# CapAI/ship-sim-gym

Hardware: AMD Instinct MI355X
Metric: env steps/sec (batched ShipEnv) (higher is better)
Workload: dtype f64

## Files before the change

ship_sim_gym_amd/csrc/shipsim_kernels.hip:

```cpp
#include <hip/hip_runtime.h>

#include <cfloat>
#include <cstdint>
#include <type_traits>

#include "shipsim.h"
#include "shipsim_internal.h"

namespace ssg {

__device__ __forceinline__ double *lds_base()
{
    extern __shared__ double s_lds[];
    return s_lds;
}

__device__ __forceinline__ double dmin(double a, double b) { return __builtin_fmin(a, b); }
__device__ __forceinline__ double dmax(double a, double b) { return __builtin_fmax(a, b); }

__device__ __forceinline__ double obs_fma(double a, double b, double c)
{
#ifndef SSG_NO_LIDAR_FMA
    return __builtin_fma(a, b, c);
#else
// ... 104 lines not shown
        const double py = goal_at<LDS_BANK, DYN>(c, goff, g, 1);
        const double dx = px - x, dy = py - y;
        const double d = obs_fma(dx, dx, dy * dy);
        const bool take = ((gm >> g) & 1u) & (d < best);
        best = take ? d : best;
        gi = take ? g : gi;
    }
    if (gi >= 0) { gx = goal_at<LDS_BANK, DYN>(c, goff, gi, 0); gy = goal_at<LDS_BANK, DYN>(c, goff, gi, 1); }
}

__device__ __forceinline__ void nearest_goal_regs(int n_goals, unsigned gm, double x, double y, const double *gp, double &gx, double &gy)
{
    gx = -1.0;
    gy = -1.0;
    double best = INFINITY;
#pragma unroll
    for (int g = 0; g < SSG_MAX_GOALS; ++g) {
        const double px = gp[2 * g], py = gp[2 * g + 1];
        const double dx = px - x, dy = py - y;
        const double d = obs_fma(dx, dx, dy * dy);
        const bool take = (g < n_goals) & (bool)((gm >> g) & 1u) & (d < best);
        best = take ? d : best;
        gx = take ? px : gx;
        gy = take ? py : gy;
    }
}

__device__ __forceinline__ int next_map(const DevCfg &c, int map_id, int env)
{
    if (c.map_ring > 0) {
        const int base = env * c.map_ring;
        const int nxt = map_id + 1;
        return (nxt - base >= c.map_ring) ? base : nxt;
    }
    const int nxt = map_id + 1;
    return (nxt >= c.n_maps) ? 0 : nxt;
}

__device__ __forceinline__ void beam_end(double cx, double cy, double ca, double sa, double cphi, double sphi, double dist,
                                         double &ex, double &ey)
{
    const double ux = obs_fma(ca, cphi, -(sa * sphi)), uy = obs_fma(sa, cphi, ca * sphi);
    ex = obs_fma(dist, ux, cx);
    ey = obs_fma(dist, uy, cy);
}

__host__ __device__ __forceinline__ constexpr int nb_lo(int nb) { return (nb + 1) / 2; }
constexpr int kBeamTabBytes = 2 * SSG_MAX_BEAMS * 8;
constexpr int kShipTabBytes = 6 * 8 * 8;
constexpr int kTrafficTabBytes = SSG_N_TRAFFIC * 4 * 8 * 8;
constexpr int kPoseDoubles = 7;
constexpr int kGoalScratchBytes = 64 * SSG_MAX_GOALS * 2 + 64 * 4;
constexpr int kTrafficScratchBytes = 64 * SSG_N_TRAFFIC * 2 + 64 * 4;
__host__ __device__ __forceinline__ constexpr int lds_fixed_bytes(int epw, bool dyn)
{
    return kBeamTabBytes + kShipTabBytes + (dyn ? kTrafficTabBytes : 0) + kPoseDoubles * epw * 8 + (dyn ? 8 : 6) * epw * 4 + 4 * (epw / 64) * 4 +
           (epw / 64) * (kGoalScratchBytes + (dyn ? kTrafficScratchBytes : 0));
}
__host__ __device__ __forceinline__ constexpr int lds_res_bytes(int nb) { return nb * 64 * 8; }
__host__ __device__ __forceinline__ constexpr int lds_queue_bytes(int nb0) { return (2 * nb0 * 64 + 64) * 2; }
__host__ __device__ __forceinline__ constexpr int lds_tile_bytes(int nb)
{
    return 2 * lds_res_bytes(nb) + 2 * lds_queue_bytes(nb_lo(nb));
}

constexpr int kHdrLidar = 10, kHdrGoals = 2 * SSG_MAX_GOALS;
static_assert(SSG_MAP_OFF_COUNTS == 0 && SSG_MAP_OFF_AABB == 2 && SSG_MAP_OFF_GOALS == kHdrLidar && SSG_MAP_OFF_SPAWN_GOAL == kHdrLidar + kHdrGoals,
              "the record's head: counts, boxes, goals, spawn goal");
#ifndef SSG_SIX_ROLE_MAX_EPW
#define SSG_SIX_ROLE_MAX_EPW 128
#endif
__host__ __device__ __forceinline__ constexpr int tile_roles(int epw, bool dyn) { return (epw <= SSG_SIX_ROLE_MAX_EPW && !dyn) ? 6 : 4; }
__host__ __device__ __forceinline__ constexpr int lds_hdr_bytes(int epw, bool lds_bank, bool dyn) { return lds_bank ? 0 : ((tile_roles(epw, dyn) - 2) * kHdrLidar + kHdrGoals) * epw * 8; }

constexpr unsigned long long kLidarMiss = ~0ull;

template <bool LDS_BANK> struct PlaneChunk { static constexpr int n = LDS_BANK ? 4 : 8; };

template <bool EXACT>
__device__ __forceinline__ double seg_mad(double a, double b, double c) { return EXACT ? a * b + c : obs_fma(a, b, c); }

template <bool LDS_BANK, bool EXACT>
__device__ __forceinline__ void lidar_pass(const DevCfg &c, const int n_items, const unsigned short *queue,
                                           unsigned long long *res , const double *beamtab,
                                           const double cx, const double cy, const double ca, const double sa,
                                           const int rec_off, const int lane, const double *hLt = nullptr , const int ld = 0)
{
    for (int base = 0; base < n_items; base += 64) {
        const int idx = base + lane;
        const bool act = idx < n_items;
        const unsigned code = queue[act ? idx : 0];
        const int src = code & 63, bi = (code >> 6) & (SSG_MAX_BEAMS - 1), s = (code >> 10) & 1;
        const double wcx = __shfl(cx, src), wcy = __shfl(cy, src), wca = __shfl(ca, src), wsa = __shfl(sa, src);
        const int woff = __shfl(rec_off, src);
        double ex, ey;
        beam_end(wcx, wcy, wca, wsa, beamtab[bi], beamtab[SSG_MAX_BEAMS + bi], c.lidar_dist, ex, ey);
        int cnt;
        if constexpr (LDS_BANK) cnt = (int)bank_at<LDS_BANK>(c, woff + SSG_MAP_OFF_COUNTS + s);
        else cnt = (int)hLt[s * ld + src];
        const int pb = woff + SSG_MAP_OFF_PLANES + s * (SSG_MAX_HULL * SSG_PLANE_DOUBLES);
        bool outside = false;
        bool out_sure = false, maybe = false;
        constexpr double kSignEps = 1e-9;
        bool ok = false;
        double ptx = ex, pty = ey;
        double bd = -1.0, bden = 1.0, t_hit = 0.0;
        int bj = 0;
        constexpr int kPlaneChunk = PlaneChunk<LDS_BANK>::n;
        for (int j0 = 0; __any(act & (j0 < cnt)); j0 += kPlaneChunk) {
            double pv0x[kPlaneChunk], pv0y[kPlaneChunk], pnx[kPlaneChunk], pny[kPlaneChunk], pv0n[kPlaneChunk];
            double pdtmin[kPlaneChunk], pdtmax[kPlaneChunk];
#pragma unroll
            for (int u = 0; u < kPlaneChunk; ++u) {
                const int j = j0 + u;
                const int q = pb + SSG_PLANE_DOUBLES * ((j < SSG_MAX_HULL) ? j : 0);
                const bool want = LDS_BANK || (act & (j < cnt));
                pv0x[u] = pv0y[u] = pnx[u] = pny[u] = pv0n[u] = 0.0;
                if (EXACT && want) { const double2 vv = bank_at2<LDS_BANK>(c, q + 0); pv0x[u] = vv.x; pv0y[u] = vv.y; }
                if (want) { const double2 nn = bank_at2<LDS_BANK>(c, q + 2); pnx[u] = nn.x; pny[u] = nn.y; }
                if (want) pv0n[u] = bank_at<LDS_BANK>(c, q + 4);
                if (EXACT) {
                    const int jp = (j == 0) ? cnt - 1 : j - 1;
                    const int qp = pb + SSG_PLANE_DOUBLES * ((jp >= 0 && jp < SSG_MAX_HULL) ? jp : 0);
                    const double ux = bank_at<LDS_BANK>(c, qp + 0), uy = bank_at<LDS_BANK>(c, qp + 1);
                    pdtmin[u] = seg_mad<EXACT>(pnx[u], uy, -(pny[u] * ux));
// ... 463 lines not shown
            const bool frontB = (snx_ * v0x + sny_ * v0y) > off_i;
            const unsigned long long mV = __ballot(valid);
            const unsigned long long mA = __ballot(valid & frontA);
            const unsigned long long missB = mV & ~__ballot(valid & frontB);
            const unsigned long long P = 0x0084210842108421ull;
            const unsigned long long allA = mA & (mA >> 1) & (mA >> 2) & (mA >> 3) & (mA >> 4) & P;
            bool sepB = false;
#pragma unroll
            for (int i = 0; i < SSG_SHIP_VERTS; ++i) sepB = sepB | (((missB >> i) & P) == 0ull);
            const bool separated = (allA != 0ull) | sepB;
            col = col | !separated;
        }
        colliding = (lane == src) ? col : colliding;
    }
    return colliding;
}

template <int NB, int EPW, bool LDS_BANK, bool EXACT, bool DYN>
__global__ __launch_bounds__(tile_roles(EPW, DYN) * EPW) void step_kernel(const DevCfg c, const int32_t *__restrict__ actions_kn,
                                                       double *__restrict__ obs, double *__restrict__ reward_out,
                                                       uint8_t *__restrict__ done_out, uint8_t *__restrict__ flags_out,
                                                       const int K_launch, const long long traj)
{
    const int K = DYN ? 1 : K_launch;
    SSG_CLOCK_BEGIN();
    constexpr int NB0 = nb_lo(NB);
    constexpr int NR = tile_roles(EPW, DYN);
    const int role = threadIdx.x / EPW;
    const int tl = threadIdx.x - role * EPW;
    const int e = blockIdx.x * EPW + tl;
    const bool live = e < c.n_envs;
    const int el_ = live ? e : 0;
    const size_t np = (size_t)c.n_pad;
    const int lane = threadIdx.x & 63;

    double *__restrict__ colX = c.f64cols + COL_X * np;
    double *__restrict__ colY = c.f64cols + COL_Y * np;
    double *__restrict__ colVX = c.f64cols + COL_VX * np;
    double *__restrict__ colVY = c.f64cols + COL_VY * np;
    double *__restrict__ colA = c.f64cols + COL_A * np;
    double *__restrict__ colW = c.f64cols + COL_W * np;
    double *__restrict__ colCum = c.f64cols + COL_CUM * np;
    double *__restrict__ colLid = c.f64cols + COL_LIDAR * np;
    int32_t *__restrict__ colRud = c.i32cols + ICOL_RUDDER * np;
    int32_t *__restrict__ colStep = c.i32cols + ICOL_STEP * np;
    int32_t *__restrict__ colMap = c.i32cols + ICOL_MAP * np;

    const int bank_bytes = LDS_BANK ? ((c.n_maps * (SSG_MAP_STRIDE * 8) + 15) & ~15) : 0;
    char *lds_fixed = reinterpret_cast<char *>(lds_base()) + bank_bytes;
    double *beamtab = reinterpret_cast<double *>(lds_fixed);
    double *shiptab = reinterpret_cast<double *>(lds_fixed + kBeamTabBytes);
    double *traffictab = reinterpret_cast<double *>(lds_fixed + kBeamTabBytes + kShipTabBytes);
    double *pose = reinterpret_cast<double *>(lds_fixed + kBeamTabBytes + kShipTabBytes + (DYN ? kTrafficTabBytes : 0));
    int *posem = reinterpret_cast<int *>(pose + kPoseDoubles * EPW);
    int *poser = posem + EPW;
    unsigned *gres = reinterpret_cast<unsigned *>(poser + EPW);
    unsigned *gdone = gres + 2 * EPW;
    unsigned *gtraf = gdone + 2 * EPW;
    unsigned *sync_ready = gtraf + (DYN ? 2 * EPW : 0);
    unsigned *sync_ack = sync_ready + EPW / 64;
    unsigned *sync_bar = sync_ack + EPW / 64;
    char *goal_scratch0 = reinterpret_cast<char *>(sync_bar + 2 * (EPW / 64));
    char *traffic_scratch0 = goal_scratch0 + (EPW / 64) * kGoalScratchBytes;
    char *scratch0 = lds_fixed + lds_fixed_bytes(EPW, DYN);
    char *tile_base = scratch0 + (tl >> 6) * lds_tile_bytes(NB);
    double *hdr0 = reinterpret_cast<double *>(scratch0 + (EPW / 64) * lds_tile_bytes(NB));
    double *hL = LDS_BANK ? nullptr : hdr0 + ((role & 1) + (role >= 4 ? 2 : 0)) * (kHdrLidar * EPW) + tl;
    double *hG = LDS_BANK ? nullptr : hdr0 + (NR - 2) * kHdrLidar * EPW + tl;
    auto load_hdr_lidar = [&](int rec_off) {
#pragma unroll
        for (int f = 0; f < kHdrLidar / 2; ++f) { const double2 v = bank_at2<LDS_BANK>(c, rec_off + 2 * f); hL[(2 * f) * EPW] = v.x; hL[(2 * f + 1) * EPW] = v.y; }
    };
    auto load_hdr_goals = [&](int rec_off) {
#pragma unroll
        for (int f = 0; f < kHdrGoals / 2; ++f) { const double2 v = bank_at2<LDS_BANK>(c, rec_off + SSG_MAP_OFF_GOALS + 2 * f); hG[(2 * f) * EPW] = v.x; hG[(2 * f + 1) * EPW] = v.y; }
    };

#ifdef SSG_STAMPS
    unsigned long long stamp_[16] = {};
#endif
    SSG_STAMP(8);

    double bank_tail_v = 0.0;
    int bank_tail_o = -1;
    if (LDS_BANK && !SSG_ABL(8)) stage_bank_lds<NR * EPW>(c.bank, c.n_maps * (SSG_MAP_STRIDE * 8), bank_tail_v, bank_tail_o);
    double tv[6] = {0.0, 0.0, 0.0, 0.0, 0.0, 0.0};
    if (threadIdx.x < 2 * SSG_MAX_BEAMS)
        tv[0] = (threadIdx.x < SSG_MAX_BEAMS) ? c.beam_cos[threadIdx.x & (SSG_MAX_BEAMS - 1)] : c.beam_sin[threadIdx.x & (SSG_MAX_BEAMS - 1)];
    if (threadIdx.x >= 64 && threadIdx.x < 64 + SSG_SHIP_VERTS) {
        const int i = threadIdx.x - 64, ip = (i == 0) ? (SSG_SHIP_VERTS - 1) : (i - 1);
        tv[0] = c.hull[2 * i]; tv[1] = c.hull[2 * i + 1]; tv[2] = c.nrm[2 * i]; tv[3] = c.nrm[2 * i + 1]; tv[4] = c.hull[2 * ip]; tv[5] = c.hull[2 * ip + 1];
    }
    if constexpr (DYN) {
        if (threadIdx.x >= 160 && threadIdx.x < 160 + SSG_N_TRAFFIC * SSG_SHIP_VERTS) {
            const int kk = (threadIdx.x - 160) / SSG_SHIP_VERTS, i = (threadIdx.x - 160) % SSG_SHIP_VERTS;
            tv[0] = c.thull[kk][2 * i]; tv[1] = c.thull[kk][2 * i + 1]; tv[2] = c.tnrm[kk][2 * i]; tv[3] = c.tnrm[kk][2 * i + 1];
        }
    }
    auto flush_tables = [&]() {
        if (bank_tail_o >= 0) *reinterpret_cast<double *>(reinterpret_cast<char *>(lds_base()) + bank_tail_o) = bank_tail_v;
        if (threadIdx.x < 2 * SSG_MAX_BEAMS) beamtab[threadIdx.x] = tv[0];
        if (threadIdx.x >= 64 && threadIdx.x < 64 + SSG_SHIP_VERTS) {
            const int i = threadIdx.x - 64;
            shiptab[0 * 8 + i] = tv[0]; shiptab[1 * 8 + i] = tv[1];
            shiptab[2 * 8 + i] = tv[2]; shiptab[3 * 8 + i] = tv[3];
            shiptab[4 * 8 + i] = tv[4]; shiptab[5 * 8 + i] = tv[5];
        }
        if constexpr (DYN) {
            if (threadIdx.x >= 160 && threadIdx.x < 160 + SSG_N_TRAFFIC * SSG_SHIP_VERTS) {
                const int kk = (threadIdx.x - 160) / SSG_SHIP_VERTS, i = (threadIdx.x - 160) % SSG_SHIP_VERTS;
                traffictab[(kk * 4 + 0) * 8 + i] = tv[0]; traffictab[(kk * 4 + 1) * 8 + i] = tv[1];
                traffictab[(kk * 4 + 2) * 8 + i] = tv[2]; traffictab[(kk * 4 + 3) * 8 + i] = tv[3];
            }
        }
    };
    if (threadIdx.x == 128) {
        double bl = INFINITY, br = -INFINITY, bb = INFINITY, bt = -INFINITY;
        for (int i = 0; i < SSG_SHIP_VERTS; ++i) {
            const double hx = c.hull[2 * i], hy = c.hull[2 * i + 1];
            const double wx = 1.0 * hx + (-0.0) * hy + c.spawn_x, wy = 0.0 * hx + 1.0 * hy + c.spawn_y;
            bl = dmin(bl, wx); br = dmax(br, wx); bb = dmin(bb, wy); bt = dmax(bt, wy);
        }
        shiptab[0 * 8 + 6] = c.spawn_x + (br - bl) / 2;
        shiptab[1 * 8 + 6] = c.spawn_y + (bt - bb) / 2;
    }
    if (threadIdx.x >= 192 && threadIdx.x < 192 + 4 * (EPW / 64)) sync_ready[threadIdx.x - 192] = 0u;
    const bool auto_reset = (c.flags & SSG_FLAG_AUTO_RESET) != 0u;
    const int tile = tl >> 6;
    auto wait_pose = [&](int k) {
        while (__hip_atomic_load(&sync_ready[tile], __ATOMIC_ACQUIRE, __HIP_MEMORY_SCOPE_WORKGROUP) != (unsigned)(k + 1))
            __builtin_amdgcn_s_sleep(2);
    };
    auto ack_pose = [&]() {
        if (lane == 0) __hip_atomic_fetch_add(&sync_ack[tile], 1u, __ATOMIC_RELEASE, __HIP_MEMORY_SCOPE_WORKGROUP);
    };
    unsigned *sync_q = sync_bar + EPW / 64;
    auto query_done = [&]() {
        if (lane == 0) __hip_atomic_fetch_add(&sync_q[tile], 1u, __ATOMIC_RELEASE, __HIP_MEMORY_SCOPE_WORKGROUP);
    };
    auto wait_queries = [&]() {
        while (__hip_atomic_load(&sync_q[tile], __ATOMIC_ACQUIRE, __HIP_MEMORY_SCOPE_WORKGROUP) < 2u)
            __builtin_amdgcn_s_sleep(1);
    };
    auto tile_barrier = [&](int k) {
        if (lane == 0) __hip_atomic_fetch_add(&sync_bar[tile], 1u, __ATOMIC_RELEASE, __HIP_MEMORY_SCOPE_WORKGROUP);
        while (__hip_atomic_load(&sync_bar[tile], __ATOMIC_ACQUIRE, __HIP_MEMORY_SCOPE_WORKGROUP) < (unsigned)NR * (unsigned)(k + 1))
            __builtin_amdgcn_s_sleep(1);
    };

    auto traffic_collide = [&](auto k0_, auto k1_, const double *tpre, double x, double y, double ca, double sa, int part,
                               unsigned short *tq , unsigned *tw ) {
        constexpr int K0 = decltype(k0_)::value, K1 = decltype(k1_)::value;
        const int wq = lane / 5, wi = lane - 5 * wq;
        const double w_hx = shiptab[0 * 8 + wi], w_hy = shiptab[1 * 8 + wi], w_nx = shiptab[2 * 8 + wi], w_ny = shiptab[3 * 8 + wi];
        double sbl, sbr, sbb, sbt;
        {
            double swx[SSG_SHIP_VERTS], swy[SSG_SHIP_VERTS];
            ship_world(shiptab, ca, sa, x, y, swx, swy, sbl, sbr, sbb, sbt);
        }
        tw[lane] = 0u;
        int n_tp = 0;
#pragma unroll
        for (int kk = K0; kk < K1; ++kk) {
            const double tx = tpre[4 * kk + 0], ty = tpre[4 * kk + 1];
            const double dx = dmax(dmax(sbl - tx, tx - sbr), 0.0), dy = dmax(dmax(sbb - ty, ty - sbt), 0.0);
            bool cand = false;
            if (live & ((dx * dx + dy * dy) <= c.dyn_reach2[kk])) {
                const double tca = tpre[4 * kk + 2], tsa = tpre[4 * kk + 3];
                double bl = INFINITY, br = -INFINITY, bb = INFINITY, bt = -INFINITY;
#pragma unroll
                for (int i = 0; i < SSG_SHIP_VERTS; ++i) {
                    const double gx = traffictab[(kk * 4 + 0) * 8 + i], gy = traffictab[(kk * 4 + 1) * 8 + i];
                    const double wx = tca * gx + (-tsa) * gy + tx, wy = tsa * gx + tca * gy + ty;
                    bl = dmin(bl, wx); br = dmax(br, wx); bb = dmin(bb, wy); bt = dmax(bt, wy);
                }
                cand = (sbl <= br) & (bl <= sbr) & (sbb <= bt) & (bb <= sbt);
            }
            const unsigned long long m = __ballot(cand);
            const int pos = n_tp + (int)__builtin_amdgcn_mbcnt_hi((unsigned)(m >> 32), __builtin_amdgcn_mbcnt_lo((unsigned)m, 0u));
            if (cand) tq[pos] = (unsigned short)(lane | (kk << 6));
            n_tp += __popcll(m);
        }
        for (int base = 0; base < n_tp; base += 12) {
            const int p = base + wq;
            const bool valid = (lane < 60) & (p < n_tp);
            const unsigned code = tq[valid ? p : 0];
            const int src = code & 63, kk = code >> 6;
            const double bx = __shfl(x, src), by = __shfl(y, src), bca = __shfl(ca, src), bsa = __shfl(sa, src);
            double tx = __shfl(tpre[4 * K0 + 0], src), ty = __shfl(tpre[4 * K0 + 1], src), tca = __shfl(tpre[4 * K0 + 2], src), tsa = __shfl(tpre[4 * K0 + 3], src);
#pragma unroll
            for (int h = K0 + 1; h < K1; ++h) {
                const double a0 = __shfl(tpre[4 * h + 0], src), a1 = __shfl(tpre[4 * h + 1], src);
                const double a2 = __shfl(tpre[4 * h + 2], src), a3 = __shfl(tpre[4 * h + 3], src);
                tx = (kk == h) ? a0 : tx; ty = (kk == h) ? a1 : ty; tca = (kk == h) ? a2 : tca; tsa = (kk == h) ? a3 : tsa;
            }
            const double *tt = traffictab + kk * 32;
            bool sep;
            {
                const double nx = bca * w_nx + (-bsa) * w_ny, ny = bsa * w_nx + bca * w_ny;
                const double vx_ = bca * w_hx + (-bsa) * w_hy + bx, vy_ = bsa * w_hx + bca * w_hy + by;
                const double off = nx * vx_ + ny * vy_;
                double mn = INFINITY;
// ... 25 lines not shown
        }
        gtraf[part * EPW + tl] = (tw[lane] != 0u) ? 1u : 0u;
    };
    auto traffic_hit = [&](int) -> unsigned { return gtraf[tl] | gtraf[EPW + tl]; };
    if (role < 2) {
        unsigned short *queue = reinterpret_cast<unsigned short *>(tile_base + 2 * lds_res_bytes(NB) + role * lds_queue_bytes(NB0));
        const int b_first = role ? NB0 : 0, b_count = role ? (NB - NB0) : NB0;
        double ca, sa, cx, cy;
        int map_id;
        double tpre[DYN ? 4 * SSG_N_TRAFFIC : 1] = {};
        {
            const double x = colX[el_], y = colY[el_], ang = colA[el_];
            map_id = colMap[el_];
            if constexpr (!LDS_BANK) load_hdr_lidar(map_id * SSG_MAP_STRIDE);
            { const double2 sc = sincos_call(ang); sa = sc.x; ca = sc.y; }
            if (role == 0) { pose[2 * EPW + tl] = ca; pose[3 * EPW + tl] = sa; }
            flush_tables();
            if (LDS_BANK) __builtin_amdgcn_s_waitcnt(0);
            __syncthreads();
            SSG_STAMP(9);
            if constexpr (DYN) {
                {
                    const double *tcol = c.dyn_f64 + (size_t)DC_TRAFFIC * np, *trot = c.dyn_f64 + (size_t)DC_TROT * np;
#pragma unroll
                    for (int kk = 0; kk < SSG_N_TRAFFIC; ++kk) {
                        if ((kk == 0) != (role == 0)) continue;
                        tpre[4 * kk + 0] = tcol[(size_t)(9 * kk) * np + el_]; tpre[4 * kk + 1] = tcol[(size_t)(9 * kk + 1) * np + el_];
                        tpre[4 * kk + 2] = trot[(size_t)(2 * kk) * np + el_]; tpre[4 * kk + 3] = trot[(size_t)(2 * kk + 1) * np + el_];
                    }
                }
            }
            double swx[SSG_SHIP_VERTS], swy[SSG_SHIP_VERTS], bl, br, bb, bt;
            ship_world(shiptab, ca, sa, x, y, swx, swy, bl, br, bb, bt);
            cx = x + (br - bl) / 2;
            cy = y + (bt - bb) / 2;
        }
        lidar_query<NB, LDS_BANK, EXACT>(c, reinterpret_cast<unsigned long long *>(tile_base), queue, beamtab, b_first, b_count,
                                         cx, cy, ca, sa, map_id * SSG_MAP_STRIDE, live, lane, hL, EPW);
        if (K == 1) query_done();
        for (int k = 0; k < K; ++k) {
            if constexpr (NR == 4) wait_pose(k);
            if constexpr (DYN) {
#pragma unroll
                for (int i = 0; i < 4 * SSG_N_TRAFFIC; ++i) asm volatile("" : "+v"(tpre[i]));
            }
            SSG_STAMP_K(0);
            double nca = 0.0, nsa = 0.0, ncx = 0.0, ncy = 0.0, npx = 0.0, npy = 0.0;
            int nmap = 0;
            if constexpr (NR == 4) {
                nca = pose[2 * EPW + tl]; nsa = pose[3 * EPW + tl];
                ncx = pose[4 * EPW + tl]; ncy = pose[5 * EPW + tl];
                npx = pose[0 * EPW + tl]; npy = pose[1 * EPW + tl];
                nmap = posem[tl];
                ack_pose();
                reinterpret_cast<unsigned short *>(gres)[2 * ((k & 1) * EPW + tl) + role] =
                        bank_narrowphase<LDS_BANK>(c, shiptab, npx, npy, nca, nsa, nmap * SSG_MAP_STRIDE, live, lane, role, hL, EPW) ? 1 : 0;
            }
            SSG_STAMP_K(4);
            if constexpr (DYN) {
                static_assert(lds_queue_bytes(1) >= 64 * 2 + 64 * 4, "lidar-lo's pair queue holds ship 0's pair queue and hit words");
                unsigned short *tq1 = reinterpret_cast<unsigned short *>(traffic_scratch0 + (tl >> 6) * kTrafficScratchBytes);
                if (role == 0) traffic_collide(std::integral_constant<int, 0>{}, std::integral_constant<int, 1>{}, tpre, npx, npy, nca, nsa, 0,
                                               queue, reinterpret_cast<unsigned *>(queue + 64));
                else traffic_collide(std::integral_constant<int, 1>{}, std::integral_constant<int, SSG_N_TRAFFIC>{}, tpre, npx, npy, nca, nsa, 1,
                                     tq1, reinterpret_cast<unsigned *>(tq1 + 64 * SSG_N_TRAFFIC));
            }

            SSG_STAMP_K(3);
            tile_barrier(k);
            SSG_STAMP_K(1);
            if constexpr (NR == 6) {
                if (k + 1 < K) {
                    nca = pose[2 * EPW + tl]; nsa = pose[3 * EPW + tl];
                    ncx = pose[4 * EPW + tl]; ncy = pose[5 * EPW + tl];
                    nmap = posem[tl];
                    ack_pose();
                }
            }
            if (k + 1 < K) {
                const bool rs = auto_reset & ((gres[(k & 1) * EPW + tl] | (gdone[(k & 1) * EPW + tl] & 1u) | (DYN ? traffic_hit(k) : 0u)) != 0u);
                ca = rs ? 1.0 : nca; sa = rs ? 0.0 : nsa;
                cx = rs ? shiptab[0 * 8 + 6] : ncx; cy = rs ? shiptab[1 * 8 + 6] : ncy;
                map_id = rs ? next_map(c, nmap, el_) : nmap;
                if constexpr (!LDS_BANK) {
                    if (rs) load_hdr_lidar(map_id * SSG_MAP_STRIDE);
                }
                lidar_query<NB, LDS_BANK, EXACT>(c, reinterpret_cast<unsigned long long *>(tile_base + ((k + 1) & 1) * lds_res_bytes(NB)),
                                                 queue, beamtab, b_first, b_count, cx, cy, ca, sa, map_id * SSG_MAP_STRIDE, live, lane, hL, EPW);
                if (k + 1 == K - 1) query_done();
            }
            SSG_STAMP_K(2);
        }
        if (K == 1 && live) {
            const bool rs = auto_reset & ((gres[tl] | (gdone[tl] & 1u) | (DYN ? traffic_hit(0) : 0u)) != 0u);
            const unsigned long long *rk = reinterpret_cast<const unsigned long long *>(tile_base);
            for (int kb = 0; kb < b_count; ++kb) {
                const int i = b_first + kb;
                const unsigned long long key = rk[i * 64 + lane];
                const double hitd = __longlong_as_double((long long)(key & 0x7FFFFFFFFFFFFFFFull));
                if (rs | (key != kLidarMiss)) st_out(&colLid[(size_t)i * np + el_], rs ? -1.0 : hitd);
            }
        }
        SSG_STAMP(10);
        SSG_STAMP_FLUSH(3);
        SSG_CLOCK_END();
        return;
    }

    if constexpr (NR == 6) {
// ... 56 lines not shown
            for (int i = 0; i < NB; ++i) asm volatile("" : "+v"(pv[6 + i]));
            if constexpr (DYN) asm volatile("" : "+v"(pv[4]), "+v"(pv[5]));
            int map0_ = map0; unsigned gm0_ = gm0;
            asm volatile("" : "+v"(map0_), "+v"(gm0_));
            gm_pre = gm0_;
            flush_tables();
            if (LDS_BANK) __builtin_amdgcn_s_waitcnt(0);
            __syncthreads();
            SSG_STAMP(9);
            if constexpr (!DYN)
                nearest_goal<LDS_BANK, false>(c, map0_ * SSG_MAP_STRIDE + SSG_MAP_OFF_GOALS, gm0_, pv[0], pv[1], pv[4], pv[5], hG, EPW);
        }
        const bool hist2 = c.history >= 2;
        ObsTile<NB> ot;
        ot.init(lane);
        constexpr int kObsPasses = (2 * F + ObsTile<NB>::CP - 1) / ObsTile<NB>::CP;
        constexpr bool kPairs = (NB >= 8) && (NB % 2 == 0);
        constexpr bool kSplitOk = kPairs || (F % ObsTile<NB>::CP) == 0;
        const bool split_last = kSplitOk && hist2 && c.history == 2 && !SSG_ABL(7);
        for (int k = 0; k < K; ++k) {
            const bool early = split_last && (k == K - 1);
            if constexpr (kSplitOk) {
                if (early) {
                    int tw = __builtin_amdgcn_readfirstlane(tl >> 6);
                    int te0 = blockIdx.x * EPW + 64 * tw;
                    asm volatile("" : "+s"(tw), "+s"(te0));
                    double *colbuf = reinterpret_cast<double *>(scratch0 + tw * lds_tile_bytes(NB) + ((k + 1) & 1) * lds_res_bytes(NB));
                    double *__restrict__ ob = obs + ((size_t)te0 + (size_t)k * (size_t)traj) * (size_t)(2 * F);
                    if constexpr (kPairs)
                        write_obs_pairs<NB, true, 0, F>(colbuf, [&](int j) -> double { return pv[(j < F) ? j : 0]; }, ob, min(64, c.n_envs - te0), lane);
                    else
                        write_obs_tile<NB, true, 0, F / ObsTile<NB>::CP>(ot, colbuf, [&](int j) -> double { return pv[(j < F) ? j : 0]; }, ob,
                                                                        min(64, c.n_envs - te0), lane);
                }
            }
            if constexpr (DYN) {
#pragma unroll
                for (int g = 0; g < SSG_MAX_GOALS; ++g) {
                    const bool listed = g < c.n_goals;
                    ogp[2 * g] = listed ? goal_at<LDS_BANK, DYN>(c, el_, g, 0) : 0.0;
                    ogp[2 * g + 1] = listed ? goal_at<LDS_BANK, DYN>(c, el_, g, 1) : 0.0;
                }
            }
            wait_pose(k);
            if constexpr (DYN) {
#pragma unroll
                for (int g = 0; g < 2 * SSG_MAX_GOALS; ++g) asm volatile("" : "+v"(ogp[g]));
            }
            SSG_STAMP_K(0);
            const double x = pose[0 * EPW + tl], y = pose[1 * EPW + tl];
            const double ang = pose[6 * EPW + tl];
            const int rudder = poser[tl];
            const int map_id = posem[tl];
            ack_pose();
            const int rec_off = map_id * SSG_MAP_STRIDE;
            SSG_STAMP_K(1);
#ifdef SSG_NO_SPEC
            const bool spec = false;
#else
            const bool spec = kSplitOk && NR == 4 && early && !SSG_ABL(7);
#endif
            double sp_gx = 0.0, sp_gy = 0.0;
            if (kSplitOk && spec) {
                wait_queries();
                const unsigned listed_pre = gm_pre & ((1u << c.n_goals) - 1u);
                if constexpr (DYN) nearest_goal_regs(c.n_goals, listed_pre, x, y, ogp, sp_gx, sp_gy);
                else nearest_goal<LDS_BANK, false>(c, rec_off + SSG_MAP_OFF_GOALS, listed_pre, x, y, sp_gx, sp_gy, hG, EPW);
                double sv[F];
                sv[0] = x; sv[1] = y; sv[2] = (double)rudder; sv[3] = ang; sv[4] = sp_gx; sv[5] = sp_gy;
                int tw = __builtin_amdgcn_readfirstlane(tl >> 6);
                int te0 = blockIdx.x * EPW + 64 * tw;
                asm volatile("" : "+s"(tw), "+s"(te0));
                const unsigned long long *rk = reinterpret_cast<const unsigned long long *>(scratch0 + tw * lds_tile_bytes(NB) + (k & 1) * lds_res_bytes(NB));
#pragma unroll
                for (int i = 0; i < NB; ++i) {
                    const unsigned long long key = rk[i * 64 + lane];
                    const double hitd = __longlong_as_double((long long)(key & 0x7FFFFFFFFFFFFFFFull));
                    sv[6 + i] = (key == kLidarMiss) ? pv[6 + i] : hitd;
                }
                double *colbuf = reinterpret_cast<double *>(scratch0 + tw * lds_tile_bytes(NB) + ((k + 1) & 1) * lds_res_bytes(NB));
                double *__restrict__ ob = obs + ((size_t)te0 + (size_t)k * (size_t)traj) * (size_t)(2 * F);
                if constexpr (kPairs)
                    write_obs_pairs<NB, true, F, 2 * F>(colbuf, [&](int j) -> double { return sv[(j < F) ? 0 : j - F]; }, ob, min(64, c.n_envs - te0), lane);
                else
                    write_obs_tile<NB, true, kSplitOk ? F / ObsTile<NB>::CP : 0, kObsPasses>(ot, colbuf, [&](int j) -> double {
                        return sv[(j < F) ? 0 : j - F]; }, ob, min(64, c.n_envs - te0), lane);
            }
            tile_barrier(k);
            SSG_STAMP_K(2);

            const unsigned gd = gdone[(k & 1) * EPW + tl];
            const bool colliding = (gres[(k & 1) * EPW + tl] != 0u) | (DYN && traffic_hit(k) != 0u);
            const bool do_reset = auto_reset & (colliding | ((gd & 1u) != 0u));
            if (live && k < K - 1) {
                const bool goal_reached = (gd & 4u) != 0u;
                double rew = goal_reached ? 1.0 : ((gd & 8u) ? -1.0 : -0.01);
                if ((c.flags & SSG_FLAG_FIX_COLLISION_REWARD) && (colliding & !goal_reached)) rew = -1.0;
                const size_t eo = (size_t)el_ + (size_t)k * (size_t)traj;
                st_out(&reward_out[eo], rew);
                st_out(&done_out[eo], (uint8_t)((colliding | ((gd & 1u) != 0u)) ? 1 : 0));
                if (flags_out) {
                    unsigned ev = 0;
                    if (colliding) ev |= SSG_EV_COLLIDING;
                    if (goal_reached) ev |= SSG_EV_GOAL_REACHED;
                    if (gd & 8u) ev |= SSG_EV_OUT_OF_BOUNDS;
                    if (gd & 16u) ev |= SSG_EV_MAX_STEPS;
                    if (gd & 32u) ev |= SSG_EV_NO_GOALS_LEFT;
                    st_out(&flags_out[eo], (uint8_t)ev);
                }
            }
            SSG_STAMP_K(4);
            double nf_gx = sp_gx, nf_gy = sp_gy;
            if (!spec || __any((gd >> 8) != (gm_pre & ((1u << c.n_goals) - 1u)))) {
                if constexpr (DYN) nearest_goal_regs(c.n_goals, gd >> 8, x, y, ogp, nf_gx, nf_gy);
                else if (!SSG_ABL(0)) nearest_goal<LDS_BANK, false>(c, rec_off + SSG_MAP_OFF_GOALS, gd >> 8, x, y, nf_gx, nf_gy, hG, EPW);
            }
            SSG_STAMP_K(5);
            int tile_w = __builtin_amdgcn_readfirstlane(tl >> 6);
            int tile_e0 = blockIdx.x * EPW + 64 * tile_w;
            asm volatile("" : "+s"(tile_w), "+s"(tile_e0));
            char *res_k = scratch0 + tile_w * lds_tile_bytes(NB) + (k & 1) * lds_res_bytes(NB);
            const int map_new = do_reset ? next_map(c, map_id, el_) : map_id;
            double rs_gx = 0.0, rs_gy = 0.0;
            if (LDS_BANK || do_reset) {
                const double2 sg = bank_at2<LDS_BANK>(c, map_new * SSG_MAP_STRIDE + SSG_MAP_OFF_SPAWN_GOAL);
                rs_gx = sg.x; rs_gy = sg.y;
            }
            double nv[F];
            nv[0] = do_reset ? c.spawn_x : x;
            nv[1] = do_reset ? c.spawn_y : y;
            nv[2] = do_reset ? 0.0 : (double)rudder;
            nv[3] = do_reset ? 0.0 : ang;
            nv[4] = do_reset ? rs_gx : nf_gx;
            nv[5] = do_reset ? rs_gy : nf_gy;
            {
                const unsigned long long *rk = reinterpret_cast<const unsigned long long *>(res_k);
#pragma unroll
                for (int i = 0; i < NB; ++i) {
                    const unsigned long long key = rk[i * 64 + lane];
                    const double hitd = __longlong_as_double((long long)(key & 0x7FFFFFFFFFFFFFFFull));
// ... 129 lines not shown
    const double w_hx = shiptab[0 * 8 + wi], w_hy = shiptab[1 * 8 + wi];
    const double w_nx = shiptab[2 * 8 + wi], w_ny = shiptab[3 * 8 + wi];
#ifdef SSG_PRIO
    __builtin_amdgcn_s_setprio(SSG_PRIO);
#endif

    bool q_need = false;
    long long st_ret = 0;
    int st_len = 0, st_eps = 0, st_goals = 0;
    unsigned q_bucket = 0, q_arrival = 0;
    for (int k = 0; k < K; ++k) {
#ifdef SSG_STAMPS_ITER
    if (k < 8) SSG_STAMP(k);
    if (k == K - 1) SSG_STAMP(11);
    if (k == 12) SSG_STAMP(12);
    if (k == 16) SSG_STAMP(13);
#else
    SSG_STAMP_K(0);
#endif
    int el = el_;
    asm volatile("" : "+v"(el));
    const int act = act_next;
    const int rec_off = map_id * SSG_MAP_STRIDE;
    const int goff = DYN ? el_ : rec_off + SSG_MAP_OFF_GOALS;

    double fx = 0.0, fy = 0.0, tq = 0.0;
    {
        const double ca0 = pose[2 * EPW + tl], sa0 = pose[3 * EPW + tl];
        const double px = (gm & 0x80u) ? (0.0 - (double)rudder) : c.px0;
        const double py = c.py0;
        const double fwx = (-sa0) * c.force_y, fwy = ca0 * c.force_y;
        const double pwx = ca0 * px + (-sa0) * py + x, pwy = sa0 * px + ca0 * py + y;
        const double rx = pwx - x, ry = pwy - y;
        const bool thrust = act == 0;
        fx = thrust ? fwx : 0.0;
        fy = thrust ? fwy : 0.0;
        tq = thrust ? (rx * fwy - ry * fwx) : 0.0;
    }
    if (act == 1 || act == 2) {
        rudder += (act == 1) ? -c.rudder_step : c.rudder_step;
        rudder = max(-c.rudder_max, min(c.rudder_max, rudder));
        gm |= 0x80u;
    }

    x = x + vx * c.dt;
    y = y + vy * c.dt;
    ang = ang + w * c.dt;
    vx = vx * c.damp + (fx * c.m_inv) * c.dt;
    vy = vy * c.damp + (fy * c.m_inv) * c.dt;
    w = w * c.damp + tq * c.i_inv * c.dt;
    double sa, ca;
    if constexpr (DYN) {
        sincos_body(ang, &sa, &ca);
    } else {
        const double2 sc = sincos_call(ang); sa = sc.x; ca = sc.y;
    }

    double sbl, sbr, sbb, sbt;
    {
        double swx[SSG_SHIP_VERTS], swy[SSG_SHIP_VERTS];
        ship_world(shiptab, ca, sa, x, y, swx, swy, sbl, sbr, sbb, sbt);
    }
    while (__hip_atomic_load(&sync_ack[tile], __ATOMIC_ACQUIRE, __HIP_MEMORY_SCOPE_WORKGROUP) != (unsigned)(NR - 1) * (unsigned)k)
        __builtin_amdgcn_s_sleep(1);
    pose[0 * EPW + tl] = x; pose[1 * EPW + tl] = y; pose[2 * EPW + tl] = ca; pose[3 * EPW + tl] = sa;
    pose[4 * EPW + tl] = x + (sbr - sbl) / 2;
    pose[5 * EPW + tl] = y + (sbt - sbb) / 2;
    pose[6 * EPW + tl] = ang;
    posem[tl] = map_id;
    poser[tl] = rudder;
    SSG_STAMP_K(1);
    if (lane == 0) __hip_atomic_store(&sync_ready[tile], (unsigned)(k + 1), __ATOMIC_RELEASE, __HIP_MEMORY_SCOPE_WORKGROUP);
    SSG_STAMP_K(2);
    if constexpr (DYN) have_goals();

    const bool oob_x = (x < 0.0) | (x > c.width);
    const bool oob_y = (y < 0.0) | (y > c.height);

    bool goal_reached;
    {
        const double w_px = shiptab[4 * 8 + wi], w_py = shiptab[5 * 8 + wi];
        unsigned short *gq = reinterpret_cast<unsigned short *>(goal_scratch0 + (tl >> 6) * kGoalScratchBytes);
        unsigned *gw = reinterpret_cast<unsigned *>(gq + 64 * SSG_MAX_GOALS);
        gw[lane] = 0u;
        int n_pairs = 0;
        auto near_test = [&](int g, double gx, double gy) {
            const double r = c.goal_r;
            const bool near = live & !SSG_ABL(5) & (bool)((gm >> g) & 1u) & ((gx - r) <= sbr) & (sbl <= (gx + r)) &
                              ((gy - r) <= sbt) & (sbb <= (gy + r));
            const unsigned long long m = __ballot(near);
            const int pos = n_pairs + (int)__builtin_amdgcn_mbcnt_hi((unsigned)(m >> 32), __builtin_amdgcn_mbcnt_lo((unsigned)m, 0u));
            if (near) gq[pos] = (unsigned short)(lane | (g << 6));
            n_pairs += __popcll(m);
        };
        if constexpr (!LDS_BANK && !DYN) {
#pragma unroll
            for (int g = 0; g < SSG_MAX_GOALS; ++g)
                if (g < c.n_goals) near_test(g, hG[(2 * g) * EPW], hG[(2 * g + 1) * EPW]);
        } else if constexpr (DYN) {
#pragma unroll
            for (int g = 0; g < SSG_MAX_GOALS; ++g)
                if (g < c.n_goals) near_test(g, gpre[2 * g], gpre[2 * g + 1]);
        } else {
            for (int g = 0; g < c.n_goals; ++g) near_test(g, goal_at<LDS_BANK, DYN>(c, goff, g, 0), goal_at<LDS_BANK, DYN>(c, goff, g, 1));
        }
        for (int base = 0; base < n_pairs; base += 12) {
            const int p = base + wq;
            const bool valid = (lane < 60) & (p < n_pairs);
            const unsigned code = gq[valid ? p : 0];
            const int src = code & 63, g = code >> 6;
            const double bx = __shfl(x, src), by = __shfl(y, src), bca = __shfl(ca, src), bsa = __shfl(sa, src);
            const int boff = __shfl(goff, src);
            double gx, gy;
            if constexpr (!LDS_BANK && !DYN) { gx = hG[(2 * g) * EPW - lane + src]; gy = hG[(2 * g + 1) * EPW - lane + src]; }
            else if constexpr (DYN) {
                (void)boff;
                gx = __shfl(gpre[0], src); gy = __shfl(gpre[1], src);
#pragma unroll
                for (int h = 1; h < SSG_MAX_GOALS; ++h) {
                    const double hx = __shfl(gpre[2 * h], src), hy = __shfl(gpre[2 * h + 1], src);
                    gx = (g == h) ? hx : gx; gy = (g == h) ? hy : gy;
// ... 51 lines not shown
    if (do_reset) map_id = next_map(c, map_id, el_);

    if constexpr (DYN) {
        if (live) {
        }
        bool need_full = false;
        if (live) {
            bool resting = !do_reset & ((dflag & 4u) != 0u);
            if (resting & goal_reached) {
                const unsigned long long lv = dlive;
                unsigned long long gone = 0ull;
                const unsigned removed = ~gm & ((1u << c.n_goals) - 1u);
                for (int g = 0; g < c.n_goals; ++g) {
                    if (!((removed >> g) & 1u)) continue;
                    gone |= 3ull << (9 + 2 * g);
                    gone |= 7ull << (21 + 3 * g);
                    for (int h = 0; h < c.n_goals; ++h)
                        if (h != g) gone |= 1ull << (h < g ? 39 + g * (g - 1) / 2 + h : 39 + h * (h - 1) / 2 + g);
                }
                resting = (lv & gone) == 0ull;
            }
            need_full = !resting;
        }
        if (need_full) {
            const unsigned bucket = dyn_bucket_of(do_reset ? 0 : steps, map_id);
            q_bucket = bucket;
            q_arrival = atomicAdd(c.dyn_count + (size_t)(c.dyn_par ^ 1) * kDynCountWords + dyn_counter_word(bucket), 1u);
        }
        q_need = need_full;
        if (live) {
            c.dyn_flag[el_] = (uint8_t)((do_reset ? 2u : (dflag & 4u)) | (need_full ? 8u : 0u));
            if (need_full) c.dyn_qmap[el_] = map_id;
        }
    }
    SSG_STAMP_K(6);
    if (live && !SSG_ABL(6)) {
        if (done) {
            st_ret += (long long)llrint(cum * 100.0);
            st_len += steps;
            st_eps += 1;
        }
        st_goals += goal_reached ? 1 : 0;
    }
    if (do_reset) {
        episodes += 1;
        if constexpr (!LDS_BANK && !DYN) load_hdr_goals(map_id * SSG_MAP_STRIDE);
    }
    SSG_STAMP_K(7);
    if (do_reset) {
        x = c.spawn_x; y = c.spawn_y; vx = 0.0; vy = 0.0; ang = 0.0; w = 0.0; cum = 0.0;
        rudder = 0; steps = 0;
        gm = (1u << c.n_goals) - 1u;
        pose[2 * EPW + tl] = 1.0; pose[3 * EPW + tl] = 0.0;
    }
    if (k == K - 1 && live && !SSG_ABL(9)) {
        st_out(&colX[el], x); st_out(&colY[el], y); st_out(&colVX[el], vx); st_out(&colVY[el], vy); st_out(&colA[el], ang);
        st_out(&colW[el], w); st_out(&colCum[el], cum);
        st_out(&colRud[el], rudder); st_out(&colStep[el], steps); st_out(&colMap[el], map_id);
        st_out(&c.i32cols[(size_t)ICOL_EPISODE * np + el], episodes);
        st_out(&c.mask[el], (uint8_t)gm);
    }
    SSG_STAMP_K(5);
    if constexpr (DYN) {
        if (k < K - 1 && q_need && q_arrival < (unsigned)c.n_pad) c.dyn_bucket[(size_t)q_bucket * np + q_arrival] = el_;
    }
    }
    if (!SSG_ABL(6)) {
        if (__any((st_eps | st_goals) != 0)) {
            auto wave_sum = [&](int v) -> int {
                v += __builtin_amdgcn_update_dpp(0, v, 0x111, 0xF, 0xF, false);
                v += __builtin_amdgcn_update_dpp(0, v, 0x112, 0xF, 0xF, false);
                v += __builtin_amdgcn_update_dpp(0, v, 0x114, 0xF, 0xF, false);
                v += __builtin_amdgcn_update_dpp(0, v, 0x118, 0xF, 0xF, false);
                v += __builtin_amdgcn_update_dpp(0, v, 0x142, 0xA, 0xF, false);
                v += __builtin_amdgcn_update_dpp(0, v, 0x143, 0xC, 0xF, false);
                return __builtin_amdgcn_readlane(v, 63);
            };
            const unsigned long long biased = (unsigned long long)(st_ret + (1ll << 40));
            const int lo = wave_sum((int)(biased & 0xFFFFu)), mid = wave_sum((int)((biased >> 16) & 0xFFFFu)), hi = wave_sum((int)(biased >> 32));
            const int len = wave_sum(st_len), eps = wave_sum(st_eps), goals = wave_sum(st_goals);
            if (lane == 0) {
                unsigned long long *slot = reinterpret_cast<unsigned long long *>(c.stats) + 4 * (blockIdx.x % kStatsSlots);
                const long long ret = (long long)lo + ((long long)mid << 16) + ((long long)hi << 32) - 64ll * (1ll << 40);
                if (eps) {
                    atomicAdd(slot + 0, (unsigned long long)ret);
                    atomicAdd(slot + 1, (unsigned long long)(long long)len);
                    atomicAdd(slot + 2, (unsigned long long)(long long)eps);
                }
                if (goals) atomicAdd(slot + 3, (unsigned long long)(long long)goals);
            }
        }
    }
    if (live) {
        const int par = (K - 1) & 1;
        const size_t el = (size_t)el_ + (size_t)(K - 1) * (size_t)traj;
        const unsigned gd = gdone[par * EPW + tl];
        const bool colliding = (gres[par * EPW + tl] != 0u) | (DYN && traffic_hit(par) != 0u);
        const bool goal_reached = (gd & 4u) != 0u;
        double rew = goal_reached ? 1.0 : ((gd & 8u) ? -1.0 : -0.01);
        if ((c.flags & SSG_FLAG_FIX_COLLISION_REWARD) && (colliding & !goal_reached)) rew = -1.0;
        st_out(&reward_out[el], rew);
        st_out(&done_out[el], (uint8_t)((colliding | ((gd & 1u) != 0u)) ? 1 : 0));
        if (flags_out) {
            unsigned ev = 0;
            if (colliding) ev |= SSG_EV_COLLIDING;
            if (goal_reached) ev |= SSG_EV_GOAL_REACHED;
// ... 238 lines not shown
```

Measured before the change: 13.12 billion.

## Hand off next-step sincos computation to a helper wave role

For non-dynamic configurations with four tile roles, the physics role now publishes next step's angle (ang + w*dt) to LDS. A helper role (role 2 by default) computes sincos of it in parallel and writes the result back, so the physics role reads the precomputed sin/cos instead of calling sincos on its critical path. Resets write the identity sin/cos. This adds LDS space and relies on the existing ack/ready ordering to make the handover safe.

```diff
diff --git a/ship_sim_gym_amd/csrc/shipsim_kernels.hip b/ship_sim_gym_amd/csrc/shipsim_kernels.hip
--- a/ship_sim_gym_amd/csrc/shipsim_kernels.hip
+++ b/ship_sim_gym_amd/csrc/shipsim_kernels.hip
@@ -180,25 +180,31 @@
 constexpr int kPoseDoubles = 7;
 constexpr int kGoalScratchBytes = 64 * SSG_MAX_GOALS * 2 + 64 * 4;
 constexpr int kTrafficScratchBytes = 64 * SSG_N_TRAFFIC * 2 + 64 * 4;
-__host__ __device__ __forceinline__ constexpr int lds_fixed_bytes(int epw, bool dyn)
-{
-    return kBeamTabBytes + kShipTabBytes + (dyn ? kTrafficTabBytes : 0) + kPoseDoubles * epw * 8 + (dyn ? 8 : 6) * epw * 4 + 4 * (epw / 64) * 4 +
-           (epw / 64) * (kGoalScratchBytes + (dyn ? kTrafficScratchBytes : 0));
-}
-__host__ __device__ __forceinline__ constexpr int lds_res_bytes(int nb) { return nb * 64 * 8; }
-__host__ __device__ __forceinline__ constexpr int lds_queue_bytes(int nb0) { return (2 * nb0 * 64 + 64) * 2; }
-__host__ __device__ __forceinline__ constexpr int lds_tile_bytes(int nb)
-{
-    return 2 * lds_res_bytes(nb) + 2 * lds_queue_bytes(nb_lo(nb));
-}
-
-constexpr int kHdrLidar = 10, kHdrGoals = 2 * SSG_MAX_GOALS;
-static_assert(SSG_MAP_OFF_COUNTS == 0 && SSG_MAP_OFF_AABB == 2 && SSG_MAP_OFF_GOALS == kHdrLidar && SSG_MAP_OFF_SPAWN_GOAL == kHdrLidar + kHdrGoals,
-              "the record's head: counts, boxes, goals, spawn goal");
 #ifndef SSG_SIX_ROLE_MAX_EPW
 #define SSG_SIX_ROLE_MAX_EPW 128
 #endif
 __host__ __device__ __forceinline__ constexpr int tile_roles(int epw, bool dyn) { return (epw <= SSG_SIX_ROLE_MAX_EPW && !dyn) ? 6 : 4; }
+#ifdef SSG_NO_SINCOS_HANDOVER
+constexpr bool kSincosHandover = false;
+#else
+constexpr bool kSincosHandover = true;
+#endif
+__host__ __device__ __forceinline__ constexpr int handover_doubles(int epw, bool dyn) { return (kSincosHandover && !dyn && tile_roles(epw, dyn) == 4) ? 3 : 0; }
+__host__ __device__ __forceinline__ constexpr int lds_fixed_bytes(int epw, bool dyn)
+{
+    return kBeamTabBytes + kShipTabBytes + (dyn ? kTrafficTabBytes : 0) + (kPoseDoubles + handover_doubles(epw, dyn)) * epw * 8 + (dyn ? 8 : 6) * epw * 4 + 4 * (epw / 64) * 4 +
+           (epw / 64) * (kGoalScratchBytes + (dyn ? kTrafficScratchBytes : 0));
+}
+__host__ __device__ __forceinline__ constexpr int lds_res_bytes(int nb) { return nb * 64 * 8; }
+__host__ __device__ __forceinline__ constexpr int lds_queue_bytes(int nb0) { return (2 * nb0 * 64 + 64) * 2; }
+__host__ __device__ __forceinline__ constexpr int lds_tile_bytes(int nb)
+{
+    return 2 * lds_res_bytes(nb) + 2 * lds_queue_bytes(nb_lo(nb));
+}
+
+constexpr int kHdrLidar = 10, kHdrGoals = 2 * SSG_MAX_GOALS;
+static_assert(SSG_MAP_OFF_COUNTS == 0 && SSG_MAP_OFF_AABB == 2 && SSG_MAP_OFF_GOALS == kHdrLidar && SSG_MAP_OFF_SPAWN_GOAL == kHdrLidar + kHdrGoals,
+              "the record's head: counts, boxes, goals, spawn goal");
 __host__ __device__ __forceinline__ constexpr int lds_hdr_bytes(int epw, bool lds_bank, bool dyn) { return lds_bank ? 0 : ((tile_roles(epw, dyn) - 2) * kHdrLidar + kHdrGoals) * epw * 8; }
 
 constexpr unsigned long long kLidarMiss = ~0ull;
@@ -768,7 +774,9 @@
     double *shiptab = reinterpret_cast<double *>(lds_fixed + kBeamTabBytes);
     double *traffictab = reinterpret_cast<double *>(lds_fixed + kBeamTabBytes + kShipTabBytes);
     double *pose = reinterpret_cast<double *>(lds_fixed + kBeamTabBytes + kShipTabBytes + (DYN ? kTrafficTabBytes : 0));
-    int *posem = reinterpret_cast<int *>(pose + kPoseDoubles * EPW);
+    double *ang_next_col = pose + kPoseDoubles * EPW;
+    double *sc_next = ang_next_col + EPW;
+    int *posem = reinterpret_cast<int *>(pose + (kPoseDoubles + handover_doubles(EPW, DYN)) * EPW);
     int *poser = posem + EPW;
     unsigned *gres = reinterpret_cast<unsigned *>(poser + EPW);
     unsigned *gdone = gres + 2 * EPW;
@@ -864,6 +872,17 @@
             __builtin_amdgcn_s_sleep(1);
     };
 
+    constexpr bool kHand = handover_doubles(EPW, DYN) != 0;
+#ifndef SSG_SINCOS_HELPER
+#define SSG_SINCOS_HELPER 2
+#endif
+    constexpr int kHelper = SSG_SINCOS_HELPER;
+    auto hand_over = [&](double an) {
+        const double2 sc = sincos_call(an);
+        sc_next[tl] = sc.x; sc_next[EPW + tl] = sc.y;
+    };
+    (void)hand_over; (void)ang_next_col; (void)kHelper;
+
     auto traffic_collide = [&](auto k0_, auto k1_, const double *tpre, double x, double y, double ca, double sa, int part,
                                unsigned short *tq , unsigned *tw ) {
         constexpr int K0 = decltype(k0_)::value, K1 = decltype(k1_)::value;
@@ -995,9 +1014,12 @@
                 ncx = pose[4 * EPW + tl]; ncy = pose[5 * EPW + tl];
                 npx = pose[0 * EPW + tl]; npy = pose[1 * EPW + tl];
                 nmap = posem[tl];
+                const bool helps = kHand && kHelper == 0 && role == 0 && k + 1 < K;
+                const double an = helps ? ang_next_col[tl] : 0.0;
                 ack_pose();
                 reinterpret_cast<unsigned short *>(gres)[2 * ((k & 1) * EPW + tl) + role] =
                         bank_narrowphase<LDS_BANK>(c, shiptab, npx, npy, nca, nsa, nmap * SSG_MAP_STRIDE, live, lane, role, hL, EPW) ? 1 : 0;
+                if (helps) hand_over(an);
             }
             SSG_STAMP_K(4);
             if constexpr (DYN) {
@@ -1160,9 +1182,12 @@
             const double ang = pose[6 * EPW + tl];
             const int rudder = poser[tl];
             const int map_id = posem[tl];
+            const bool helps = kHand && kHelper == 2 && k + 1 < K;
+            const double an = helps ? ang_next_col[tl] : 0.0;
             ack_pose();
             const int rec_off = map_id * SSG_MAP_STRIDE;
             SSG_STAMP_K(1);
+            if (helps) hand_over(an);
 #ifdef SSG_NO_SPEC
             const bool spec = false;
 #else
@@ -1194,6 +1219,7 @@
                     write_obs_tile<NB, true, kSplitOk ? F / ObsTile<NB>::CP : 0, kObsPasses>(ot, colbuf, [&](int j) -> double {
                         return sv[(j < F) ? 0 : j - F]; }, ob, min(64, c.n_envs - te0), lane);
             }
+            SSG_STAMP_K(12);
             tile_barrier(k);
             SSG_STAMP_K(2);
 
@@ -1429,6 +1455,8 @@
     double sa, ca;
     if constexpr (DYN) {
         sincos_body(ang, &sa, &ca);
+    } else if (kHand && k > 0) {
+        sa = sc_next[tl]; ca = sc_next[EPW + tl];
     } else {
         const double2 sc = sincos_call(ang); sa = sc.x; ca = sc.y;
     }
@@ -1444,6 +1472,9 @@
     pose[4 * EPW + tl] = x + (sbr - sbl) / 2;
     pose[5 * EPW + tl] = y + (sbt - sbb) / 2;
     pose[6 * EPW + tl] = ang;
+    if constexpr (kHand) {
+        if (k + 1 < K) ang_next_col[tl] = ang + w * c.dt;
+    }
     posem[tl] = map_id;
     poser[tl] = rudder;
     SSG_STAMP_K(1);
@@ -1601,6 +1632,7 @@
         rudder = 0; steps = 0;
         gm = (1u << c.n_goals) - 1u;
         pose[2 * EPW + tl] = 1.0; pose[3 * EPW + tl] = 0.0;
+        if constexpr (kHand) { sc_next[tl] = 0.0; sc_next[EPW + tl] = 1.0; }
     }
     if (k == K - 1 && live && !SSG_ABL(9)) {
         st_out(&colX[el], x); st_out(&colY[el], y); st_out(&colVX[el], vx); st_out(&colVY[el], vy); st_out(&colA[el], ang);
```

Result: slower. 12.88 billion (-1.8%).
